# MuellerNico/DD2360-RayTracing

Hardware: AMD Instinct MI355X
Metric: Msamples/s (W*H*spp/render_time) at 1200x800, 10000 spheres (higher is better)
Workload: dtype f32

## Files before the change

dd2360-raytracing_amd/csrc/rt_kernels.hip:

```cpp
#include <hip/hip_runtime.h>
#include <float.h>
#include "rt_device.h"
#include "rt_tuning.h"
#include "rt_sampling.h"
#include "rt_sched_keep.h"

#ifdef RT_TU_CONTRACT
#pragma clang fp contract(fast)
#else
#pragma clang fp contract(off)
#endif

namespace rt {
#ifdef RT_TU_CONTRACT
namespace fmac {
#endif

#define RT_DEV static __device__ __forceinline__

#include "rt_stats.h"

struct Rng { uint32_t d, v0, v1, v2, v3, v4; };

RT_DEV float rng_uniform(Rng& s) {
// ... 185 lines not shown
                const float mn = group_min<64>(my_t);
                const int km = wave_min_int((my_t == mn && my_k != 0x7fffffff) ? my_k : 0x7fffffff);
                if (lane == L && km != 0x7fffffff && mn < closest) { closest = mn; best = T.ent_id[km]; }
            }
            return;
        }
    }
    int e_best = -1;
    int node = live ? 0 : T.n_nodes;
    const int n_nodes = T.n_nodes;
    while (true) {
        int e = 0, e_end = 0;
        while (node < n_nodes) {
            const float4 n0 = s_nodes[node * 3 + 0];
            const float4 n1 = s_nodes[node * 3 + 1];
            const float4 n2 = s_nodes[node * 3 + 2];
            const int skip = __float_as_int(n1.z);
            if (ray_box(r, n0.x, n0.y, n0.z, n0.w, n1.x, n1.y)) {
                const int cnt = __float_as_int(n2.x);
                node = node + 1;
                if (cnt > 0) { e = __float_as_int(n1.w); e_end = e + cnt; break; }
            } else {
                node = skip;
            }
        }
        if (e >= e_end) break;
        while (e < e_end) {
            const int m = e_end - e;
            const float4 s0 = T.ent_hot[e], s1 = T.ent_hot[m > 1 ? e + 1 : e], s2 = T.ent_hot[m > 2 ? e + 2 : e], s3 = T.ent_hot[m > 3 ? e + 3 : e];
            sphere_test(r, a, s0.x, s0.y, s0.z, s0.w, e, closest, e_best);
            if (m > 1) sphere_test(r, a, s1.x, s1.y, s1.z, s1.w, e + 1, closest, e_best);
            if (m > 2) sphere_test(r, a, s2.x, s2.y, s2.z, s2.w, e + 2, closest, e_best);
            if (m > 3) sphere_test(r, a, s3.x, s3.y, s3.z, s3.w, e + 3, closest, e_best);
            e += m > 4 ? 4 : m;
        }
    }
    if (e_best >= 0) best = T.ent_id[e_best];
}

RT_DEV bool eligible(const float4* s_nodes, const RayF& r, float cand, int sphere STAT_ARG) {
    const DevTree& T = cold_args()->tree;
    STAT(st, ST_ELIG, 1); WPASS(WP_ELIG_FN);
    {
        const int row = T.acc.bits_index[sphere];
        const float px = r.o.x + cand * r.d.x, py = r.o.y + cand * r.d.y, pz = r.o.z + cand * r.d.z;
        const int ix = (int)floorf((px + kRootHalfXZf) * kInvCellXZf), iy = (int)floorf(py * kInvCellYf), iz = (int)floorf((pz + kRootHalfXZf) * kInvCellXZf);
        if (row >= 0 && ix >= 0 && ix < 8 && iy >= 0 && iy < 8 && iz >= 0 && iz < 8) {
            const int cell = ix * 64 + iy * 8 + iz;
            const int node = T.acc.cellnode[cell];
            const uint32_t word = T.acc.cellbits[row * 16 + (cell >> 5)];
            if (node >= 0 && ((word >> (cell & 31)) & 1u)) {
                const float4 n0 = s_nodes[node * 3 + 0];
                const float4 n1 = s_nodes[node * 3 + 1];
                const float m = 0.012f;
                if (px > n0.x + m && px < n0.w - m && py > n0.y + m && py < n1.x - m && pz > n0.z + m && pz < n1.y - m) return true;
            }
        }
    }
    const int mb = T.acc.memb_start[sphere], me = T.acc.memb_start[sphere + 1];
    for (int k = mb; k < me; ++k) {
        const int node = T.acc.memb_cell[k];
        STAT(st, ST_ELIG_NODES, 1); WPASS(WP_ELIG_LIST);
        const float4 n0 = s_nodes[node * 3 + 0];
        const float4 n1 = s_nodes[node * 3 + 1];
        if (ray_box(r, n0.x, n0.y, n0.z, n0.w, n1.x, n1.y)) return true;
    }
    return false;
}

RT_DEV bool in_brick(const RayF& r, float cand, const float4 blo, const float4 bhi) {
    const float ux = __builtin_fmaf(__builtin_fmaf(cand, r.d.x, r.o.x), kInvCellXZf, 4.0f);
    const float uy = __builtin_fmaf(cand, r.d.y, r.o.y) * kInvCellYf;
    const float uz = __builtin_fmaf(__builtin_fmaf(cand, r.d.z, r.o.z), kInvCellXZf, 4.0f);
    return ux > blo.x && ux < bhi.x && uy > blo.y && uy < bhi.y && uz > blo.z && uz < bhi.z;
}

RT_DEV void offer(const DevTree& T, const float4* s_nodes, const RayF& r, float cand, const float4 blo, const float4 bhi, float& best_t, int& best, bool& tie STAT_ARG) {
    STAT(st, ST_OFFERS, 1);
    const int id = __float_as_int(blo.w);
    if (cand < best_t) {
        bool ok = in_brick(r, cand, blo, bhi);
        if (!ok) {
            const int node1 = __float_as_int(bhi.w);
            if (node1 >= 0) {
                STAT(st, ST_ELIG, 1); STAT(st, ST_ELIG_NODES, 1); WPASS(WP_OFFER_RAYBOX);
                const float4 n0 = s_nodes[node1 * 3 + 0];
                const float4 n1 = s_nodes[node1 * 3 + 1];
                ok = ray_box(r, n0.x, n0.y, n0.z, n0.w, n1.x, n1.y);
            } else {
                ok = eligible(s_nodes, r, cand, id STAT_PASS);
            }
        }
        if (ok) { best_t = cand; best = id; }
    } else if (cand == best_t && id != best && best > 0) {
        tie = true;
    }
}

struct Walk {
    int i, iend, coff;
    float om_c, on_c, slope, dm_c;
    bool fwd, walking;
    unsigned work, cols;
};

RT_DEV void walk_clip(Walk& W, const DevAccel& A, float best_t) {
    const float fG = (float)A.G, back_c = 2e-3f * A.inv_h;
    const float pm = fminf(fmaxf(W.om_c + best_t * W.dm_c, -4.0f), fG + 4.0f);
    if (W.fwd) W.iend = min(W.iend, (int)floorf(pm + back_c) + 1);
    else W.iend = max(W.iend, (int)ceilf(pm - back_c - 1.0f) - 1);
    if (W.fwd ? (W.i >= W.iend) : (W.i <= W.iend)) W.i = W.iend;
}

RT_DEV Walk walk_setup(const DevAccel& A, const RayF& r, float best_t, int best) {
    Walk W;
    W.work = 0u; W.cols = 0u;
    const int G = A.G;
    const float fG = (float)G;
    const float slack = 2e-3f;
    const bool xmajor = fabsf(r.d.x) >= fabsf(r.d.z);
    const float om = xmajor ? r.o.x : r.o.z, on = xmajor ? r.o.z : r.o.x;
    const float dm = xmajor ? r.d.x : r.d.z, dn = xmajor ? r.d.z : r.d.x;
    W.coff = xmajor ? 0 : A.zoff;
    W.om_c = (om - A.g0) * A.inv_h; W.on_c = (on - A.g0) * A.inv_h;
    W.dm_c = dm * A.inv_h;
    const float s_c = slack * A.inv_h;
    const float rmy = W.dm_c * __builtin_amdgcn_rcpf(r.d.y);
    const float mA = W.om_c + (A.ylo - r.o.y) * rmy, mB = W.om_c + (A.yhi - r.o.y) * rmy;
    float mlo = fminf(mA, mB) - s_c, mhi = fmaxf(mA, mB) + s_c;
    W.fwd = dm > 0.0f;
    if (W.fwd) mlo = fmaxf(mlo, W.om_c - s_c); else mhi = fminf(mhi, W.om_c + s_c);
    int ilo = (int)floorf(fminf(fmaxf(mlo, -1.0f), fG)), ihi = (int)floorf(fminf(fmaxf(mhi, -1.0f), fG));
    W.walking = !(ihi < 0 || ilo > G - 1 || !(mlo <= mhi));
    ilo = max(ilo, 0); ihi = min(ihi, G - 1);
    W.i = W.fwd ? ilo : ihi;
    W.iend = (W.fwd ? ihi : ilo) + (W.fwd ? 1 : -1);
    W.slope = dn * __builtin_amdgcn_rcpf(dm);
    if (best >= 0) walk_clip(W, A, best_t);
    if (W.i == W.iend || (W.fwd ? (W.i > W.iend) : (W.i < W.iend))) W.walking = false;
    return W;
}

static_assert(RT_POOL_COLS_THIN >= RT_POOL_COLS, "a thin round takes at least as many columns as a full one");
constexpr int kWalkPool = 64 * RT_POOL_COLS;
constexpr int kWalkCand = 128;
struct WalkLds {
    uint2 seg[kWalkPool];
    unsigned pref[kWalkPool];
    float4 ray[128];
    unsigned long long key[64];
    uint4 cq[kWalkCand];
    unsigned count, tie_lo, tie_hi, pad_;
};
struct PoolSpan { unsigned cur, end, seg_end, base, sg; int owner; RayF q; float a, abt, atm; };
RT_DEV void walk_sync() { __builtin_amdgcn_fence(__ATOMIC_SEQ_CST, "wavefront"); __builtin_amdgcn_wave_barrier(); }
RT_DEV unsigned walk_excl_scan(unsigned v, unsigned& total) {
    int x = (int)v;
    x += __builtin_amdgcn_update_dpp(0, x, 0x111, 0xf, 0xf, false);
    x += __builtin_amdgcn_update_dpp(0, x, 0x112, 0xf, 0xf, false);
    x += __builtin_amdgcn_update_dpp(0, x, 0x114, 0xf, 0xf, false);
    x += __builtin_amdgcn_update_dpp(0, x, 0x118, 0xf, 0xf, false);
    x += __builtin_amdgcn_update_dpp(0, x, 0x142, 0xa, 0xf, false);
    x += __builtin_amdgcn_update_dpp(0, x, 0x143, 0xc, 0xf, false);
    total = (unsigned)__builtin_amdgcn_readlane(x, 63);
    return (unsigned)x - v;
}

RT_DEV void pool_candidate_b(const DevTree& T, const float4* s_nodes, WalkLds& L, const uint4 c, const float4 blo, const float4 bhi STAT_ARG) {
    const int owner = (int)c.w;
    const float b = __uint_as_float(c.x), disc = __uint_as_float(c.y);
    const float4 r0 = L.ray[2 * owner], r1 = L.ray[2 * owner + 1];
    RayF q; q.o = {r0.x, r0.y, r0.z}; q.d = {r0.w, r1.x, r1.y};
    const float a = r1.z;
    const unsigned long long k0 = L.key[owner];
    const float best_t = __uint_as_float((unsigned)(k0 >> 32));
    const int best = (int)(unsigned)k0;
    const float sq = sqrtf(disc);
    float cand = __builtin_inff();
    const float t1 = (-b - sq) / a;
    if (t1 > 0.001f) cand = t1;
    else { const float t2 = (-b + sq) / a; if (t2 > 0.001f) cand = t2; }
    if (!(cand <= best_t)) return;
    const int id = __float_as_int(blo.w);
    STAT(st, ST_OFFERS, 1);
    bool tie = false;
    if (cand < best_t) {
        bool ok = in_brick(q, cand, blo, bhi);
        if (!ok) {
            const int node1 = __float_as_int(bhi.w);
            if (node1 >= 0) {
                const float4 n0 = s_nodes[node1 * 3 + 0], n1 = s_nodes[node1 * 3 + 1];
                ok = ray_box(q, n0.x, n0.y, n0.z, n0.w, n1.x, n1.y);
            } else ok = eligible(s_nodes, q, cand, id STAT_PASS);
        }
        if (ok) {
            const unsigned long long old = atomicMin(&L.key[owner], ((unsigned long long)__float_as_uint(cand) << 32) | (unsigned)id);
            tie = (unsigned)(old >> 32) == __float_as_uint(cand) && (int)(unsigned)old != id && (int)(unsigned)old > 0;
        }
    } else tie = id != best && best > 0;
    if (tie) { if (owner < 32) atomicOr(&L.tie_lo, 1u << owner); else atomicOr(&L.tie_hi, 1u << (owner - 32)); }
}

RT_DEV void pool_candidate(const DevTree& T, const float4* s_nodes, WalkLds& L, const uint4 c STAT_ARG) {
    const int e = (int)c.z;
    const float4 blo = T.acc.brick[2 * e], bhi = T.acc.brick[2 * e + 1];
    pool_candidate_b(T, s_nodes, L, c, blo, bhi STAT_PASS);
}

RT_DEV void pool_drain(const DevTree& T, const float4* s_nodes, WalkLds& L, int lane, unsigned& qn STAT_ARG) {
    walk_sync();
    const unsigned cnt = min(qn, (unsigned)kWalkCand);
    for (unsigned base = 0; base < cnt; base += 64u) {
        STAT(st, ST_B_ROUNDS_WAVE, 1);
        const unsigned i = base + (unsigned)lane;
        if (i < cnt) { STAT(st, ST_B_LANES, 1); pool_candidate(T, s_nodes, L, L.cq[i] STAT_PASS); }
    }
    qn = 0u;
    walk_sync();
}

template <int RT_QUORUM_DEN>
RT_DEV void walk_pool(const DevTree& T, const float4* s_nodes, WalkLds& L, const RayF& r, float a, Walk& W, float& best_t, int& best, bool& tie STAT_ARG) {
    const DevAccel& A = T.acc;
    const int32_t* __restrict__ cs = A.cs;
    const float4* __restrict__ hot = A.hot;
    const int lane = threadIdx.x & 63;
    const int Gf = A.Gf;
    const float fF = (float)A.F, fGf = (float)Gf, fGfm = fGf - 0.5f, q_c = A.rq_c;
    const int step = W.fwd ? 1 : -1;
    const float f_atm = a * (0.001f * 0.9999f - 1e-6f);
    bool walking = W.walking && W.i != W.iend;
    const int nw0 = __popcll(__ballot(walking));
    L.ray[2 * lane] = make_float4(r.o.x, r.o.y, r.o.z, r.d.x);
    while (true) {
        L.ray[2 * lane + 1] = make_float4(r.d.y, r.d.z, a, __builtin_fmaf(a * best_t, 1.0001f, 1e-6f * a));
        L.key[lane] = ((unsigned long long)__float_as_uint(best_t) << 32) | (unsigned)best;
        if (lane == 0) { L.tie_lo = 0u; L.tie_hi = 0u; }
        walk_sync();
        const int cols_now = nw0 * RT_POOL_COLS_THIN <= kWalkPool ? RT_POOL_COLS_THIN : RT_POOL_COLS;
        int e0[RT_POOL_COLS_THIN], e1[RT_POOL_COLS_THIN];
#pragma unroll
        for (int c = 0; c < RT_POOL_COLS_THIN; ++c) {
            e0[c] = 0; e1[c] = 0;
            if (c < cols_now && walking && W.i != W.iend) {
                STAT(st, ST_COLS, 1);
                const float u0 = W.on_c + ((float)W.i - W.om_c) * W.slope, u1 = u0 + W.slope;
                const float lo = (fminf(u0, u1) - q_c) * fF, hi = (fmaxf(u0, u1) + q_c) * fF;
                if (hi >= 0.0f && lo < fGf) {
                    const int k0 = (int)fmaxf(lo, 0.0f), k1 = (int)fminf(hi, fGfm);
                    const unsigned cbase = (unsigned)(W.coff + W.i * Gf);
                    e0[c] = cs[cbase + (unsigned)k0]; e1[c] = cs[cbase + (unsigned)k1 + 1u];
                }
                W.i += step; ++W.cols;
            }
        }
        unsigned n_seg = 0u;
#pragma unroll
        for (int c = 0; c < RT_POOL_COLS_THIN; ++c) {
            if (c >= RT_POOL_COLS && c >= cols_now) break;
            const bool has = e1[c] > e0[c];
            const unsigned long long m = __ballot(has);
            if (has) {
                const unsigned slot = n_seg + __builtin_amdgcn_mbcnt_hi((unsigned)(m >> 32), __builtin_amdgcn_mbcnt_lo((unsigned)m, 0u));
                L.seg[slot] = make_uint2((unsigned)e0[c], (unsigned)(e1[c] - e0[c]) | ((unsigned)lane << 26));
                W.work += (unsigned)(e1[c] - e0[c]);
            }
            n_seg += (unsigned)__popcll(m);
        }
        walk_sync();
        if (n_seg != 0u) {
            unsigned total = 0u;
            {
                unsigned run = 0u;
#pragma unroll
                for (int k = 0; k < RT_POOL_COLS; ++k) {
                    const unsigned sidx = (unsigned)(k * 64 + lane);
                    const unsigned cnt = sidx < n_seg ? (L.seg[sidx].y & 0x3ffffffu) : 0u;
                    unsigned tot;
                    const unsigned ex = walk_excl_scan(cnt, tot);
                    if (sidx < n_seg) L.pref[sidx] = run + ex;
                    run += tot;
                }
                total = run;
            }
            walk_sync();
            const unsigned C = (total + 64u * RT_POOL_SPANS - 1u) / (64u * RT_POOL_SPANS);
            PoolSpan sp[RT_POOL_SPANS];
#pragma unroll
            for (int j = 0; j < RT_POOL_SPANS; ++j) {
                PoolSpan& S = sp[j];
                const unsigned begin = min((unsigned)(lane + 64 * j) * C, total);
                S.end = min(begin + C, total); S.cur = begin; S.seg_end = begin; S.base = 0u; S.sg = 0u; S.owner = -1;
                S.q.o = {0.f, 0.f, 0.f}; S.q.d = {0.f, 1.f, 0.f}; S.a = 1.0f; S.abt = 0.0f; S.atm = 0.0f;
                if (n_seg <= 4u) {
                    const unsigned p1 = L.pref[min(1u, n_seg - 1u)], p2 = L.pref[min(2u, n_seg - 1u)], p3 = L.pref[min(3u, n_seg - 1u)];
                    S.sg = (n_seg > 1u && p1 <= begin ? 1u : 0u) + (n_seg > 2u && p2 <= begin ? 1u : 0u) + (n_seg > 3u && p3 <= begin ? 1u : 0u);
                } else if (begin < S.end) {
                    unsigned lo = 0u, hi = n_seg;
#pragma unroll
                    for (int it = 0; it < 8; ++it) {
                        const unsigned mid = (lo + hi) >> 1;
                        if (hi - lo > 1u) { if (L.pref[mid] <= begin) lo = mid; else hi = mid; }
                    }
                    S.sg = lo;
                }
            }
            unsigned qn = 0u;
            if (RT_POOL_DIRECT && RT_POOL_SPANS == 1 && total <= 64u) {
                PoolSpan& S = sp[0];
                const bool act = S.cur < S.end;
                STAT(st, ST_A_ITERS_WAVE, 1);
                unsigned he = 0u;
                if (act) {
                    const uint2 sd = L.seg[S.sg];
                    const unsigned p0 = L.pref[S.sg];
                    he = sd.x - p0 + S.cur;
                    S.owner = (int)(sd.y >> 26);
                    const float4 r0 = L.ray[2 * S.owner], r1 = L.ray[2 * S.owner + 1];
                    S.q.o = {r0.x, r0.y, r0.z}; S.q.d = {r0.w, r1.x, r1.y}; S.a = r1.z; S.abt = r1.w;
                    S.atm = S.a * (0.001f * 0.9999f - 1e-6f);
                }
                const float4 s4 = hot[he], blo = A.brick[2 * he], bhi = A.brick[2 * he + 1];
                STAT(st, ST_TESTS, act ? 1 : 0); STAT(st, ST_A_LANE_STEPS, act ? 1 : 0);
                const float ocx = S.q.o.x - s4.x, ocy = S.q.o.y - s4.y, ocz = S.q.o.z - s4.z;
                const float b = ocx * S.q.d.x + ocy * S.q.d.y + ocz * S.q.d.z;
                const float c = (ocx * ocx + ocy * ocy + ocz * ocz) - s4.w;
                const float disc = b * b - S.a * c;
                const float ab = fabsf(b);
                const float Lm = __builtin_fmaf(ab, -1e-4f, -b) - S.abt, M = __builtin_fmaf(ab, -1e-4f, b) + S.atm;
                const float P = fmaxf(Lm, M);
                if (act && disc > 0.0f && !(P > 0.0f && P * P > disc * 1.0003f)) {
                    STAT(st, ST_DISCPOS, 1);
                    pool_candidate_b(T, s_nodes, L, make_uint4(__float_as_uint(b), __float_as_uint(disc), he, (unsigned)S.owner), blo, bhi STAT_PASS);
                }
            } else
            while (true) {
                bool any = false;
#pragma unroll
                for (int j = 0; j < RT_POOL_SPANS; ++j) any = any || sp[j].cur < sp[j].end;
                if (__ballot(any) == 0ull) break;
                STAT(st, ST_A_ITERS_WAVE, 1);
                bool act[RT_POOL_SPANS]; unsigned he[RT_POOL_SPANS]; float4 s4[RT_POOL_SPANS];
#pragma unroll
                for (int j = 0; j < RT_POOL_SPANS; ++j) {
                    PoolSpan& S = sp[j];
                    act[j] = S.cur < S.end;
                    if (act[j] && S.cur >= S.seg_end) {
                        const uint2 sd = L.seg[S.sg];
                        const unsigned p0 = L.pref[S.sg];
                        ++S.sg;
                        S.seg_end = p0 + (sd.y & 0x3ffffffu);
                        S.base = sd.x - p0;
                        const int ow = (int)(sd.y >> 26);
                        if (ow != S.owner) {
                            S.owner = ow;
                            const float4 r0 = L.ray[2 * ow], r1 = L.ray[2 * ow + 1];
                            S.q.o = {r0.x, r0.y, r0.z}; S.q.d = {r0.w, r1.x, r1.y}; S.a = r1.z; S.abt = r1.w;
                            S.atm = S.a * (0.001f * 0.9999f - 1e-6f);
                        }
                    }
                    he[j] = act[j] ? S.base + S.cur : 0u;
                    s4[j] = hot[he[j]];
                }
                bool hold[RT_POOL_SPANS]; float hb[RT_POOL_SPANS], hd[RT_POOL_SPANS];
                bool anyhold = false;
#pragma unroll
                for (int j = 0; j < RT_POOL_SPANS; ++j) {
                    const PoolSpan& S = sp[j];
                    STAT(st, ST_TESTS, act[j] ? 1 : 0); STAT(st, ST_A_LANE_STEPS, act[j] ? 1 : 0);
                    const float ocx = S.q.o.x - s4[j].x, ocy = S.q.o.y - s4[j].y, ocz = S.q.o.z - s4[j].z;
                    const float b = ocx * S.q.d.x + ocy * S.q.d.y + ocz * S.q.d.z;
                    const float c = (ocx * ocx + ocy * ocy + ocz * ocz) - s4[j].w;
                    const float disc = b * b - S.a * c;
                    const float ab = fabsf(b);
                    const float Lm = __builtin_fmaf(ab, -1e-4f, -b) - S.abt, M = __builtin_fmaf(ab, -1e-4f, b) + S.atm;
                    const float P = fmaxf(Lm, M);
                    hold[j] = act[j] && disc > 0.0f && !(P > 0.0f && P * P > disc * 1.0003f);
                    hb[j] = b; hd[j] = disc;
                    anyhold = anyhold || hold[j];
                    if (act[j]) ++sp[j].cur;
                }
                if (__ballot(anyhold) != 0ull) {
#pragma unroll
                    for (int j = 0; j < RT_POOL_SPANS; ++j) {
                        const unsigned long long hm = __ballot(hold[j]);
                        if (hm != 0ull) {
                            const unsigned slot = qn + __builtin_amdgcn_mbcnt_hi((unsigned)(hm >> 32), __builtin_amdgcn_mbcnt_lo((unsigned)hm, 0u));
                            if (hold[j]) {
                                STAT(st, ST_DISCPOS, 1);
                                const uint4 ce = make_uint4(__float_as_uint(hb[j]), __float_as_uint(hd[j]), he[j], (unsigned)sp[j].owner);
                                if (slot < (unsigned)kWalkCand) L.cq[slot] = ce;
                                else pool_candidate(T, s_nodes, L, ce STAT_PASS);
                            }
                            qn += (unsigned)__popcll(hm);
                        }
                    }
                }
                if (qn >= 64u) pool_drain(T, s_nodes, L, lane, qn STAT_PASS);
            }
            pool_drain(T, s_nodes, L, lane, qn STAT_PASS);
            (void)f_atm;
            const unsigned long long k = L.key[lane];
            best_t = __uint_as_float((unsigned)(k >> 32)); best = (int)(unsigned)k;
            const unsigned tmask = lane < 32 ? L.tie_lo : L.tie_hi;
            if ((tmask >> (lane & 31)) & 1u) tie = true;
        }
        if (walking && best >= 0) walk_clip(W, A, best_t);
        walking = walking && W.i != W.iend;
        const int left = __popcll(__ballot(walking));
        if (left == 0) break;
        if (RT_QUORUM_DEN > 0 && nw0 >= RT_QUORUM_MIN && left * RT_QUORUM_DEN <= nw0) break;
    }
    W.walking = walking;
}

template <int RT_QUORUM_DEN>
RT_DEV void walk_pool_dense(const DevTree& T, const float4* s_nodes, WalkLds& L, const RayF& r, float a, Walk& W, float& best_t, int& best, bool& tie STAT_ARG) {
    constexpr int PB = RT_DENSE_PB;
    const DevAccel& A = T.acc;
    const int32_t* __restrict__ cs = A.cs;
    const float4* __restrict__ hot = A.hot;
    const int lane = threadIdx.x & 63;
    const int Gf = A.Gf;
    const float fF = (float)A.F, fGf = (float)Gf, fGfm = fGf - 0.5f, q_c = A.rq_c;
    const int step = W.fwd ? 1 : -1;
    bool walking = W.walking && W.i != W.iend;
    const int nw0 = __popcll(__ballot(walking));
    L.ray[2 * lane] = make_float4(r.o.x, r.o.y, r.o.z, r.d.x);
    while (true) {
        L.ray[2 * lane + 1] = make_float4(r.d.y, r.d.z, a, __builtin_fmaf(a * best_t, 1.0001f, 1e-6f * a));
        L.key[lane] = ((unsigned long long)__float_as_uint(best_t) << 32) | (unsigned)best;
        if (lane == 0) { L.tie_lo = 0u; L.tie_hi = 0u; }
        walk_sync();
        int e0 = 0, e1 = 0;
        if (walking && W.i != W.iend) {
            STAT(st, ST_COLS, 1);
            const float u0 = W.on_c + ((float)W.i - W.om_c) * W.slope, u1 = u0 + W.slope;
            const float lo = (fminf(u0, u1) - q_c) * fF, hi = (fmaxf(u0, u1) + q_c) * fF;
            if (hi >= 0.0f && lo < fGf) {
                const int k0 = (int)fmaxf(lo, 0.0f), k1 = (int)fminf(hi, fGfm);
                const unsigned cbase = (unsigned)(W.coff + W.i * Gf);
                e0 = cs[cbase + (unsigned)k0]; e1 = cs[cbase + (unsigned)k1 + 1u];
            }
            W.i += step; ++W.cols;
        }
        const bool has = e1 > e0;
        const unsigned long long m = __ballot(has);
        const unsigned n_seg = (unsigned)__popcll(m);
        if (has) {
            const unsigned slot = __builtin_amdgcn_mbcnt_hi((unsigned)(m >> 32), __builtin_amdgcn_mbcnt_lo((unsigned)m, 0u));
            L.seg[slot] = make_uint2((unsigned)e0, (unsigned)(e1 - e0) | ((unsigned)lane << 26));
            W.work += (unsigned)(e1 - e0);
        }
        walk_sync();
        if (n_seg != 0u) {
            unsigned total;
            {
                const unsigned cnt = (unsigned)lane < n_seg ? (L.seg[lane].y & 0x3ffffffu) : 0u;
                const unsigned ex = walk_excl_scan(cnt, total);
                if ((unsigned)lane < n_seg) L.pref[lane] = ex;
            }
            walk_sync();
            const unsigned C = (total + 63u) / 64u;
            PoolSpan S;
            const unsigned begin = min((unsigned)lane * C, total);
            S.end = min(begin + C, total); S.cur = begin; S.seg_end = begin; S.base = 0u; S.sg = 0u; S.owner = lane;
            S.q.o = {0.f, 0.f, 0.f}; S.q.d = {0.f, 1.f, 0.f}; S.a = 1.0f; S.abt = 0.0f; S.atm = 0.0f;
            if (begin < S.end) {
                unsigned lo = 0u, hi = n_seg;
#pragma unroll
                for (int it = 0; it < 6; ++it) {
                    const unsigned mid = (lo + hi) >> 1;
                    if (hi - lo > 1u) { if (L.pref[mid] <= begin) lo = mid; else hi = mid; }
                }
                S.sg = lo;
            }
            unsigned qn = 0u;
            while (true) {
                const bool act = S.cur < S.end;
                if (__ballot(act) == 0ull) break;
                STAT(st, ST_A_ITERS_WAVE, 1);
                if (act && S.cur >= S.seg_end) {
                    const uint2 sd = L.seg[S.sg];
                    const unsigned p0 = L.pref[S.sg];
                    ++S.sg;
                    S.seg_end = p0 + (sd.y & 0x3ffffffu);
                    S.base = sd.x - p0;
                    S.owner = (int)(sd.y >> 26);
                    const float4 r0 = L.ray[2 * S.owner], r1 = L.ray[2 * S.owner + 1];
                    S.q.o = {r0.x, r0.y, r0.z}; S.q.d = {r0.w, r1.x, r1.y}; S.a = r1.z;
                    S.atm = S.a * (0.001f * 0.9999f - 1e-6f);
                }
                const unsigned nb = act ? min((unsigned)PB, min(S.seg_end, S.end) - S.cur) : 0u;
                const unsigned he0 = act ? S.base + S.cur : 0u;
                const float4* __restrict__ hp = hot + he0;
                float4 s4[PB];
#pragma unroll
                for (int k = 0; k < PB; ++k) s4[k] = hp[k];
                const float bt_now = __uint_as_float((unsigned)(L.key[S.owner] >> 32));
                S.abt = __builtin_fmaf(S.a * bt_now, 1.0001f, 1e-6f * S.a);
                if (act) { STAT(st, ST_TESTS, nb); STAT(st, ST_A_LANE_STEPS, 1); }
                bool hold[PB]; float hb[PB], hd[PB];
                bool anyhold = false;
#pragma unroll
                for (int k = 0; k < PB; ++k) {
                    const float ocx = S.q.o.x - s4[k].x, ocy = S.q.o.y - s4[k].y, ocz = S.q.o.z - s4[k].z;
                    const float b = ocx * S.q.d.x + ocy * S.q.d.y + ocz * S.q.d.z;
                    const float c = (ocx * ocx + ocy * ocy + ocz * ocz) - s4[k].w;
                    const float disc = b * b - S.a * c;
                    const float ab = fabsf(b);
                    const float Lm = __builtin_fmaf(ab, -1e-4f, -b) - S.abt, M = __builtin_fmaf(ab, -1e-4f, b) + S.atm;
                    const float P = fmaxf(Lm, M);
                    hold[k] = (unsigned)k < nb && disc > 0.0f && !(P > 0.0f && P * P > disc * 1.0003f);
                    hb[k] = b; hd[k] = disc;
                    anyhold = anyhold || hold[k];
                }
                if (__ballot(anyhold) != 0ull) {
#pragma unroll
                    for (int k = 0; k < PB; ++k) {
                        const unsigned long long hm = __ballot(hold[k]);
                        if (hm != 0ull) {
                            const unsigned slot = qn + __builtin_amdgcn_mbcnt_hi((unsigned)(hm >> 32), __builtin_amdgcn_mbcnt_lo((unsigned)hm, 0u));
                            if (hold[k]) {
                                STAT(st, ST_DISCPOS, 1);
                                const uint4 ce = make_uint4(__float_as_uint(hb[k]), __float_as_uint(hd[k]), he0 + (unsigned)k, (unsigned)S.owner);
                                if (slot < (unsigned)kWalkCand) L.cq[slot] = ce;
                                else pool_candidate(T, s_nodes, L, ce STAT_PASS);
                            }
                            qn += (unsigned)__popcll(hm);
                        }
                    }
                }
                S.cur += nb;
                if (qn >= (unsigned)RT_DENSE_DRAIN) pool_drain(T, s_nodes, L, lane, qn STAT_PASS);
            }
            pool_drain(T, s_nodes, L, lane, qn STAT_PASS);
            const unsigned long long k = L.key[lane];
            best_t = __uint_as_float((unsigned)(k >> 32)); best = (int)(unsigned)k;
            const unsigned tmask = lane < 32 ? L.tie_lo : L.tie_hi;
            if ((tmask >> (lane & 31)) & 1u) tie = true;
        }
        if (walking && best >= 0) walk_clip(W, A, best_t);
        walking = walking && W.i != W.iend;
        const int left = __popcll(__ballot(walking));
        if (left == 0) break;
        if (RT_QUORUM_DEN > 0 && nw0 >= RT_QUORUM_MIN && left * RT_QUORUM_DEN <= nw0) break;
    }
    W.walking = walking;
}

constexpr int kHotLarge = 8;
constexpr int kHotSlots = 1 + 3 * kHotLarge;
RT_DEV float4* hot_spheres(const float4* s_nodes, int n_nodes) { return (float4*)((WalkLds*)(s_nodes + n_nodes * 3) + 4); }
template <bool POOL>
// ... 1348 lines not shown
```

dd2360-raytracing_amd/csrc/rt_stats.h:

```cpp
#pragma once
#ifdef RT_STATS
enum { ST_RAYS, ST_FAST, ST_SLOW, ST_TIE, ST_COLS, ST_TESTS, ST_DISCPOS, ST_OFFERS, ST_ELIG, ST_ELIG_NODES, ST_A_ITERS_WAVE, ST_B_ROUNDS_WAVE,
       ST_LOOP_ITERS_WAVE, ST_A_LANE_STEPS, ST_B_LANES, ST_SAMPLES, ST_LIVE_GE56, ST_LIVE_32, ST_LIVE_8, ST_LIVE_LT8, ST_SWITCHES,
       ST_CYC_TOTAL, ST_CYC_CLOSEST, ST_CYC_WALK_A, ST_CYC_WALK_B, ST_CYC_SCAN, ST_CYC_SHADE, ST_REALTIME,
       ST_SPARE0, ST_SPARE1, ST_SPARE2, ST_SPARE3, ST_SPARE4, ST_SPARE5, ST_SPARE6,
       WP_GROUND, WP_LARGE_K, WP_LARGE_EXACT, WP_OFFER_NODE, WP_OFFER_RAYBOX, WP_ELIG_FN, WP_ELIG_LIST, WP_SETUP, WP_A_COL, WP_A_BATCH, WP_A_HOLD,
       WP_B_OFFER, WP_B_CLIP, WP_COOP_CHUNK, WP_SCAN, WP_SC_ANY, WP_SC_LAMB, WP_SC_METAL, WP_SC_DIEL, WP_REJ_ITER, WP_PRIMARY, WP_DISK_ITER, WP_SKY, WP_ENDPIX,
       TH_GROUND, TH_LARGE_SETUP, TH_WALK, TH_SCAN, ST_N };
#ifdef RT_STATS_LIGHT
#define TICK() 0ull
#else
#define TICK() ((unsigned long long)__builtin_amdgcn_s_memtime())
#endif
__device__ unsigned long long g_stats[ST_N];
__device__ int g_pilot_dbg[1 << 20];
__device__ unsigned long long g_wave_dbg[8192 * 4];
struct Stats { unsigned int c[ST_N]; unsigned long long cyc[8]; };
#ifdef RT_STATS_LIGHT
#define STAT(st, k, v) ((void)0)
#else
#define STAT(st, k, v) ((st).c[k] += (v))
#endif
constexpr int kWpBlocks = WP_ENDPIX - WP_GROUND + 1;
__device__ unsigned long long g_wp_cls[4 * kWpBlocks];
#ifdef RT_STATS_WPASS
__shared__ int s_wp_cls[4];
#define WPASS(k) do { const int l_ = (int)(threadIdx.x & 63); if (__builtin_amdgcn_readfirstlane(l_) == l_) { atomicAdd(&g_stats[k], 1ull); \
    atomicAdd(&g_wp_cls[(s_wp_cls[(threadIdx.x >> 6) & 3] & 3) * kWpBlocks + ((k) - WP_GROUND)], 1ull); } } while (0)
#define WPASS_CLASS(c) do { const int l_ = (int)(threadIdx.x & 63); if (__builtin_amdgcn_readfirstlane(l_) == l_) s_wp_cls[(threadIdx.x >> 6) & 3] = (c); } while (0)
#else
#define WPASS(k) ((void)0)
#define WPASS_CLASS(c) ((void)0)
#endif
#define STAT_ARG , Stats& st
#define STAT_PASS , st
#define RT_STATS_ONLY(...) __VA_ARGS__
#define RT_STATS_READERS \
hipError_t read_pilot_dbg(int* out, int n) { return hipMemcpyFromSymbol(out, HIP_SYMBOL(g_pilot_dbg), sizeof(int) * (size_t)(n < (1 << 20) ? n : (1 << 20))); } \
hipError_t read_wave_dbg(unsigned long long* out) { return hipMemcpyFromSymbol(out, HIP_SYMBOL(g_wave_dbg), sizeof(unsigned long long) * 8192 * 4); } \
hipError_t read_wp_classes(unsigned long long* out, int reset) { \
    hipError_t e = hipMemcpyFromSymbol(out, HIP_SYMBOL(g_wp_cls), sizeof(unsigned long long) * 4 * kWpBlocks); \
    if (e != hipSuccess) return e; \
    if (reset) { unsigned long long z[4 * kWpBlocks] = {0}; e = hipMemcpyToSymbol(HIP_SYMBOL(g_wp_cls), z, sizeof(z)); } \
    return e; \
} \
hipError_t read_stats(unsigned long long* out, int reset) { \
    hipError_t e = hipMemcpyFromSymbol(out, HIP_SYMBOL(g_stats), sizeof(unsigned long long) * ST_N); \
    if (e != hipSuccess) return e; \
    if (reset) { unsigned long long z[ST_N] = {0}; e = hipMemcpyToSymbol(HIP_SYMBOL(g_stats), z, sizeof(z)); } \
    return e; \
}
#else
#define STAT(st, k, v) ((void)0)
#define WPASS(k) ((void)0)
#define WPASS_CLASS(c) ((void)0)
#define STAT_ARG
#define STAT_PASS
#define RT_STATS_ONLY(...)
#define RT_STATS_READERS
#endif
```

dd2360-raytracing_amd/csrc/rt_tuning.h:

```cpp
#pragma once

#ifndef RT_RENDER_WAVES
#define RT_RENDER_WAVES 4
#endif

#ifndef RT_LONG_RATE
#define RT_LONG_RATE 14
#endif
#ifndef RT_LONG_RATE_DENSE
#define RT_LONG_RATE_DENSE 20
#endif
#ifndef RT_LONG_CHECK
#define RT_LONG_CHECK 4
#endif
#ifndef RT_F_INFLIGHT
#define RT_F_INFLIGHT 1.35f
#endif
#ifndef RT_F_INFLIGHT_DENSE
#define RT_F_INFLIGHT_DENSE 1.1f
#endif

#ifndef RT_F_STATIC
#define RT_F_STATIC 1.07f
#endif
#ifndef RT_HEAD_SUM_SPARSE
#define RT_HEAD_SUM_SPARSE 1
#endif
#ifndef RT_HEAD_SUM_DENSE
#define RT_HEAD_SUM_DENSE -21
#endif
#ifndef RT_HEAD_LOAD_DENSE
#define RT_HEAD_LOAD_DENSE 3500
#endif
#ifndef RT_F_TAIL
#define RT_F_TAIL 0.15f
#endif
#ifndef RT_INTERLEAVE
#define RT_INTERLEAVE 64
#endif
#ifndef RT_INTERLEAVE_DENSE
#define RT_INTERLEAVE_DENSE 16
#endif
#ifndef RT_INTERLEAVE_SOLO
#define RT_INTERLEAVE_SOLO 1
#endif
#ifndef RT_LONG_RATE_MIN
#define RT_LONG_RATE_MIN 8
#endif
#ifndef RT_PILOT_LONG_SUM_MIN
#define RT_PILOT_LONG_SUM_MIN 120
#endif
#ifndef RT_MED_RATE
#define RT_MED_RATE 12
#endif
#ifndef RT_THIN_CAP_DEN
#define RT_THIN_CAP_DEN 4
#endif
#ifndef RT_LONG_PER_WAVE
#define RT_LONG_PER_WAVE 16
#endif
#ifndef RT_PILOT_SAMPLES
#define RT_PILOT_SAMPLES 2
#endif
#ifndef RT_PILOT_LONG_SUM
#define RT_PILOT_LONG_SUM 200
#endif
#ifndef RT_SOLO_DENSITY
#define RT_SOLO_DENSITY 1.0
#endif
#ifndef RT_PILOT_SOLO_SUM
#define RT_PILOT_SOLO_SUM 200
#endif
#ifndef RT_PILOT_CAP
#define RT_PILOT_CAP 35
#endif
#ifndef RT_SCHED_CACHE
#define RT_SCHED_CACHE 1
#endif
#ifndef RT_PROG_OWN
#define RT_PROG_OWN 64
#endif

#ifndef RT_SPLIT_WB
#define RT_SPLIT_WB 1000
#endif
#ifndef RT_SPLIT_WT
#define RT_SPLIT_WT 17
#endif
#ifndef RT_SPLIT_WC
#define RT_SPLIT_WC 0
#endif

#ifndef RT_ACCEL_FINE
#define RT_ACCEL_FINE 8
#endif
#ifndef RT_DENSE_CELL
#define RT_DENSE_CELL 0.7
#endif
#ifndef RT_SPARSE_CELL
#define RT_SPARSE_CELL 1.0
#endif

#ifndef RT_QUORUM_SPARSE
#define RT_QUORUM_SPARSE 4
#endif
#ifndef RT_QUORUM_DENSE
#define RT_QUORUM_DENSE 2
#endif
#ifndef RT_QUORUM_MIN
#define RT_QUORUM_MIN 16
#endif
#ifndef RT_POOL_COLS
#define RT_POOL_COLS 2
#endif
#ifndef RT_POOL_COLS_THIN
#define RT_POOL_COLS_THIN 4
#endif
#ifndef RT_POOL_SPANS
#define RT_POOL_SPANS 1
#endif
#ifndef RT_POOL_DIRECT
#define RT_POOL_DIRECT 1
#endif
#ifndef RT_DENSE_PB
#define RT_DENSE_PB 4
#endif
#ifndef RT_DENSE_DRAIN
#define RT_DENSE_DRAIN 32
#endif

#ifndef RT_LIST_BATCH
#define RT_LIST_BATCH 8
#endif
#ifndef RT_LIST_COOP_COST
#define RT_LIST_COOP_COST 16
#endif

#ifndef RT_H16_MINWAVES
#define RT_H16_MINWAVES 4
#endif
#ifndef RT_H16_BIG
#define RT_H16_BIG 128
#endif
#ifndef RT_H16_SMALL
#define RT_H16_SMALL 256
#endif
#ifndef RT_H16_INTERLEAVE
#define RT_H16_INTERLEAVE 64
#endif
#ifndef RT_H16_TASKS
#define RT_H16_TASKS 384
#endif
#ifndef RT_H16_PP
#define RT_H16_PP 10
#endif
#ifndef RT_H16_LONG_PER_WAVE
#define RT_H16_LONG_PER_WAVE 16
#endif
#ifndef RT_H16_LONG_RATE
#define RT_H16_LONG_RATE 14
#endif
#ifndef RT_H16_LONG_CHECK
#define RT_H16_LONG_CHECK 4
#endif
#ifndef RT_H16_THIN_CAP_DEN
#define RT_H16_THIN_CAP_DEN 4
#endif
#ifndef RT_H16_PILOT_LONG_SUM
#define RT_H16_PILOT_LONG_SUM 150
#endif
#ifndef RT_H16_PILOT_CAP
#define RT_H16_PILOT_CAP 35
#endif
```

Before: 4746.

## Add thin-round walk path spreading few walkers' columns across all lanes

When a wave has at most 16 active walkers, each walker's four grid columns are now given to separate lanes (16 walkers x 4 columns), so the cell-start lookups happen in parallel instead of each walker looping over its own columns. If the combined candidate count fits in 64, candidates are handed out one per lane and tested right away, skipping the segment/span pooling machinery. Otherwise it falls back to building segments. It also stops scanning empty second segment pages and passes ray data directly to the candidate routine. This adds LDS record traffic and extra branches, and carries a risk around correctness of the iteration bookkeeping.

```diff
diff --git a/dd2360-raytracing_amd/csrc/rt_kernels.hip b/dd2360-raytracing_amd/csrc/rt_kernels.hip
--- a/dd2360-raytracing_amd/csrc/rt_kernels.hip
+++ b/dd2360-raytracing_amd/csrc/rt_kernels.hip
@@ -361,6 +361,10 @@
     uint4 cq[kWalkCand];
     unsigned count, tie_lo, tie_hi, pad_;
 };
+constexpr int kThinWalkers = 16, kThinCols = 4;
+static_assert(kThinWalkers * kThinCols == 64, "a thin round: one lane per (walker, column)");
+static_assert(kThinCols == RT_POOL_COLS_THIN, "a thin round takes the columns a round of few walkers took before it");
+static_assert(sizeof(unsigned) * kWalkPool >= sizeof(uint4) * 2 * kThinWalkers && sizeof(uint2) * kWalkPool >= sizeof(uint2) * 64, "the thin round's records and slots live in pref and seg");
 struct PoolSpan { unsigned cur, end, seg_end, base, sg; int owner; RayF q; float a, abt, atm; };
 RT_DEV void walk_sync() { __builtin_amdgcn_fence(__ATOMIC_SEQ_CST, "wavefront"); __builtin_amdgcn_wave_barrier(); }
 RT_DEV unsigned walk_excl_scan(unsigned v, unsigned& total) {
@@ -375,12 +379,9 @@
     return (unsigned)x - v;
 }
 
-RT_DEV void pool_candidate_b(const DevTree& T, const float4* s_nodes, WalkLds& L, const uint4 c, const float4 blo, const float4 bhi STAT_ARG) {
+RT_DEV void pool_candidate_b(const DevTree& T, const float4* s_nodes, WalkLds& L, const uint4 c, const RayF& q, const float a, const float4 blo, const float4 bhi STAT_ARG) {
     const int owner = (int)c.w;
     const float b = __uint_as_float(c.x), disc = __uint_as_float(c.y);
-    const float4 r0 = L.ray[2 * owner], r1 = L.ray[2 * owner + 1];
-    RayF q; q.o = {r0.x, r0.y, r0.z}; q.d = {r0.w, r1.x, r1.y};
-    const float a = r1.z;
     const unsigned long long k0 = L.key[owner];
     const float best_t = __uint_as_float((unsigned)(k0 >> 32));
     const int best = (int)(unsigned)k0;
@@ -413,7 +414,9 @@
 RT_DEV void pool_candidate(const DevTree& T, const float4* s_nodes, WalkLds& L, const uint4 c STAT_ARG) {
     const int e = (int)c.z;
     const float4 blo = T.acc.brick[2 * e], bhi = T.acc.brick[2 * e + 1];
-    pool_candidate_b(T, s_nodes, L, c, blo, bhi STAT_PASS);
+    const float4 r0 = L.ray[2 * c.w], r1 = L.ray[2 * c.w + 1];
+    RayF q; q.o = {r0.x, r0.y, r0.z}; q.d = {r0.w, r1.x, r1.y};
+    pool_candidate_b(T, s_nodes, L, c, q, r1.z, blo, bhi STAT_PASS);
 }
 
 RT_DEV void pool_drain(const DevTree& T, const float4* s_nodes, WalkLds& L, int lane, unsigned& qn STAT_ARG) {
@@ -440,12 +443,95 @@
     const float f_atm = a * (0.001f * 0.9999f - 1e-6f);
     bool walking = W.walking && W.i != W.iend;
     const int nw0 = __popcll(__ballot(walking));
+    const bool thin_round = RT_POOL_THIN_ROUND && nw0 <= kThinWalkers;
     L.ray[2 * lane] = make_float4(r.o.x, r.o.y, r.o.z, r.d.x);
     while (true) {
         L.ray[2 * lane + 1] = make_float4(r.d.y, r.d.z, a, __builtin_fmaf(a * best_t, 1.0001f, 1e-6f * a));
         L.key[lane] = ((unsigned long long)__float_as_uint(best_t) << 32) | (unsigned)best;
         if (lane == 0) { L.tie_lo = 0u; L.tie_hi = 0u; }
+        const unsigned long long wmask = __ballot(walking);
+        if (thin_round && walking) {
+            const unsigned rank = __builtin_amdgcn_mbcnt_hi((unsigned)(wmask >> 32), __builtin_amdgcn_mbcnt_lo((unsigned)wmask, 0u));
+            uint4* rec = (uint4*)L.pref;
+            rec[2 * rank] = make_uint4((unsigned)lane, (unsigned)W.i, (unsigned)step, (unsigned)W.iend);
+            rec[2 * rank + 1] = make_uint4(__float_as_uint(W.om_c), __float_as_uint(W.on_c), __float_as_uint(W.slope), (unsigned)W.coff);
+        }
         walk_sync();
+        unsigned n_seg = 0u;
+        bool picked = false;
+        bool dealt = false;
+        if (thin_round) {
+            const int nwr = __popcll(wmask);
+            const int wk = lane >> 2, c = lane & 3;
+            int f0 = 0; unsigned cnt = 0u;
+            if (wk < nwr) {
+                const uint4* rec = (const uint4*)L.pref;
+                const uint4 ra = rec[2 * wk], rb = rec[2 * wk + 1];
+                const int wstep = (int)ra.z;
+                if (c < ((int)ra.w - (int)ra.y) * wstep) {
+                    const int wi = (int)ra.y + c * wstep;
+                    const float w_om = __uint_as_float(rb.x), w_on = __uint_as_float(rb.y), w_slope = __uint_as_float(rb.z);
+                    const float u0 = w_on + ((float)wi - w_om) * w_slope, u1 = u0 + w_slope;
+                    const float lo = (fminf(u0, u1) - q_c) * fF, hi = (fmaxf(u0, u1) + q_c) * fF;
+                    if (hi >= 0.0f && lo < fGf) {
+                        const int k0 = (int)fmaxf(lo, 0.0f), k1 = (int)fminf(hi, fGfm);
+                        const unsigned cbase = (unsigned)((int)rb.w + wi * Gf);
+                        const int a0 = cs[cbase + (unsigned)k0], a1 = cs[cbase + (unsigned)k1 + 1u];
+                        if (a1 > a0) { f0 = a0; cnt = (unsigned)(a1 - a0); }
+                    }
+                }
+            }
+            int qs = (int)cnt;
+            qs += __builtin_amdgcn_update_dpp(0, qs, 0xB1, 0xf, 0xf, false);
+            qs += __builtin_amdgcn_update_dpp(0, qs, 0x4E, 0xf, 0xf, false);
+            const unsigned rank = __builtin_amdgcn_mbcnt_hi((unsigned)(wmask >> 32), __builtin_amdgcn_mbcnt_lo((unsigned)wmask, 0u));
+            const int mywork = __builtin_amdgcn_ds_bpermute((int)((rank & 15u) << 4), qs);
+            if (walking) {
+                const int taken = min(kThinCols, (W.iend - W.i) * step);
+                STAT(st, ST_COLS, taken);
+                W.i += taken * step; W.cols += (unsigned)taken; W.work += (unsigned)mywork;
+            }
+            unsigned total;
+            const unsigned ex = walk_excl_scan(cnt, total);
+            RT_STATS_ONLY(n_seg = (unsigned)__popcll(__ballot(cnt != 0u)); TRSTAT_ROUND(lane, n_seg, total); n_seg = 0u;)
+            if (total <= 64u) {
+                dealt = true;
+                if (total != 0u) {
+                    picked = true;
+                    uint2* slot = (uint2*)L.seg;
+#pragma nounroll
+                    for (unsigned t = 0u; t < cnt; ++t) slot[ex + t] = make_uint2((unsigned)f0 + t, L.pref[8 * wk]);
+                    walk_sync();
+                    const bool act = (unsigned)lane < total;
+                    STAT(st, ST_A_ITERS_WAVE, 1);
+                    unsigned he = 0u; int owner = 0;
+                    if (act) { const uint2 sl = slot[lane]; he = sl.x; owner = (int)sl.y; }
+                    const float4 r0 = L.ray[2 * owner], r1 = L.ray[2 * owner + 1];
+                    const float4 s4 = hot[he], blo = A.brick[2 * he], bhi = A.brick[2 * he + 1];
+                    RayF q; q.o = {r0.x, r0.y, r0.z}; q.d = {r0.w, r1.x, r1.y};
+                    const float qa = r1.z, abt = r1.w, atm = qa * (0.001f * 0.9999f - 1e-6f);
+                    STAT(st, ST_TESTS, act ? 1 : 0); STAT(st, ST_A_LANE_STEPS, act ? 1 : 0);
+                    const float ocx = q.o.x - s4.x, ocy = q.o.y - s4.y, ocz = q.o.z - s4.z;
+                    const float b = ocx * q.d.x + ocy * q.d.y + ocz * q.d.z;
+                    const float cc = (ocx * ocx + ocy * ocy + ocz * ocz) - s4.w;
+                    const float disc = b * b - qa * cc;
+                    const float ab = fabsf(b);
+                    const float Lm = __builtin_fmaf(ab, -1e-4f, -b) - abt, M = __builtin_fmaf(ab, -1e-4f, b) + atm;
+                    const float P = fmaxf(Lm, M);
+                    if (act && disc > 0.0f && !(P > 0.0f && P * P > disc * 1.0003f)) {
+                        STAT(st, ST_DISCPOS, 1);
+                        pool_candidate_b(T, s_nodes, L, make_uint4(__float_as_uint(b), __float_as_uint(disc), he, (unsigned)owner), q, qa, blo, bhi STAT_PASS);
+                    }
+                    walk_sync();
+                }
+            } else {
+                const bool has = cnt != 0u;
+                const unsigned long long m = __ballot(has);
+                if (has) L.seg[__builtin_amdgcn_mbcnt_hi((unsigned)(m >> 32), __builtin_amdgcn_mbcnt_lo((unsigned)m, 0u))] = make_uint2((unsigned)f0, cnt | (L.pref[8 * wk] << 26));
+                n_seg = (unsigned)__popcll(m);
+                walk_sync();
+            }
+        } else {
         const int cols_now = nw0 * RT_POOL_COLS_THIN <= kWalkPool ? RT_POOL_COLS_THIN : RT_POOL_COLS;
         int e0[RT_POOL_COLS_THIN], e1[RT_POOL_COLS_THIN];
 #pragma unroll
@@ -463,7 +549,6 @@
                 W.i += step; ++W.cols;
             }
         }
-        unsigned n_seg = 0u;
 #pragma unroll
         for (int c = 0; c < RT_POOL_COLS_THIN; ++c) {
             if (c >= RT_POOL_COLS && c >= cols_now) break;
@@ -477,12 +562,16 @@
             n_seg += (unsigned)__popcll(m);
         }
         walk_sync();
-        if (n_seg != 0u) {
+        RT_STATS_ONLY(if (nw0 <= kThinWalkers && n_seg == 0u) TRSTAT_ROUND(lane, 0u, 0u);)
+        }
+        if (!dealt && n_seg != 0u) {
+            picked = true;
             unsigned total = 0u;
             {
                 unsigned run = 0u;
 #pragma unroll
                 for (int k = 0; k < RT_POOL_COLS; ++k) {
+                    if (k > 0 && n_seg <= 64u * (unsigned)k) break;
                     const unsigned sidx = (unsigned)(k * 64 + lane);
                     const unsigned cnt = sidx < n_seg ? (L.seg[sidx].y & 0x3ffffffu) : 0u;
                     unsigned tot;
@@ -492,6 +581,7 @@
                 }
                 total = run;
             }
+            RT_STATS_ONLY(if (nw0 <= kThinWalkers && !thin_round) TRSTAT_ROUND(lane, n_seg, total);)
             walk_sync();
             const unsigned C = (total + 64u * RT_POOL_SPANS - 1u) / (64u * RT_POOL_SPANS);
             PoolSpan sp[RT_POOL_SPANS];
@@ -540,7 +630,7 @@
                 const float P = fmaxf(Lm, M);
                 if (act && disc > 0.0f && !(P > 0.0f && P * P > disc * 1.0003f)) {
                     STAT(st, ST_DISCPOS, 1);
-                    pool_candidate_b(T, s_nodes, L, make_uint4(__float_as_uint(b), __float_as_uint(disc), he, (unsigned)S.owner), blo, bhi STAT_PASS);
+                    pool_candidate_b(T, s_nodes, L, make_uint4(__float_as_uint(b), __float_as_uint(disc), he, (unsigned)S.owner), S.q, S.a, blo, bhi STAT_PASS);
                 }
             } else
             while (true) {
@@ -609,6 +699,8 @@
             }
             pool_drain(T, s_nodes, L, lane, qn STAT_PASS);
             (void)f_atm;
+        }
+        if (picked) {
             const unsigned long long k = L.key[lane];
             best_t = __uint_as_float((unsigned)(k >> 32)); best = (int)(unsigned)k;
             const unsigned tmask = lane < 32 ? L.tie_lo : L.tie_hi;
diff --git a/dd2360-raytracing_amd/csrc/rt_stats.h b/dd2360-raytracing_amd/csrc/rt_stats.h
--- a/dd2360-raytracing_amd/csrc/rt_stats.h
+++ b/dd2360-raytracing_amd/csrc/rt_stats.h
@@ -6,7 +6,8 @@
        ST_SPARE0, ST_SPARE1, ST_SPARE2, ST_SPARE3, ST_SPARE4, ST_SPARE5, ST_SPARE6,
        WP_GROUND, WP_LARGE_K, WP_LARGE_EXACT, WP_OFFER_NODE, WP_OFFER_RAYBOX, WP_ELIG_FN, WP_ELIG_LIST, WP_SETUP, WP_A_COL, WP_A_BATCH, WP_A_HOLD,
        WP_B_OFFER, WP_B_CLIP, WP_COOP_CHUNK, WP_SCAN, WP_SC_ANY, WP_SC_LAMB, WP_SC_METAL, WP_SC_DIEL, WP_REJ_ITER, WP_PRIMARY, WP_DISK_ITER, WP_SKY, WP_ENDPIX,
-       TH_GROUND, TH_LARGE_SETUP, TH_WALK, TH_SCAN, ST_N };
+       TH_GROUND, TH_LARGE_SETUP, TH_WALK, TH_SCAN,
+       TR_ROUNDS, TR_SEG0, TR_SEG1, TR_SEG4, TR_SEG16, TR_SEGMORE, TR_LE64, ST_N };
 #ifdef RT_STATS_LIGHT
 #define TICK() 0ull
 #else
@@ -18,8 +19,12 @@
 struct Stats { unsigned int c[ST_N]; unsigned long long cyc[8]; };
 #ifdef RT_STATS_LIGHT
 #define STAT(st, k, v) ((void)0)
+#define TRSTAT_ROUND(lane, n_seg, total) ((void)0)
 #else
 #define STAT(st, k, v) ((st).c[k] += (v))
+#define TRSTAT_ROUND(lane, n_seg, total) do { if ((lane) == 0) { atomicAdd(&g_stats[TR_ROUNDS], 1ull); \
+    atomicAdd(&g_stats[(n_seg) == 0u ? TR_SEG0 : (n_seg) == 1u ? TR_SEG1 : (n_seg) <= 4u ? TR_SEG4 : (n_seg) <= 16u ? TR_SEG16 : TR_SEGMORE], 1ull); \
+    if ((total) <= 64u) atomicAdd(&g_stats[TR_LE64], 1ull); } } while (0)
 #endif
 constexpr int kWpBlocks = WP_ENDPIX - WP_GROUND + 1;
 __device__ unsigned long long g_wp_cls[4 * kWpBlocks];
diff --git a/dd2360-raytracing_amd/csrc/rt_tuning.h b/dd2360-raytracing_amd/csrc/rt_tuning.h
--- a/dd2360-raytracing_amd/csrc/rt_tuning.h
+++ b/dd2360-raytracing_amd/csrc/rt_tuning.h
@@ -116,6 +116,9 @@
 #ifndef RT_POOL_COLS_THIN
 #define RT_POOL_COLS_THIN 4
 #endif
+#ifndef RT_POOL_THIN_ROUND
+#define RT_POOL_THIN_ROUND 1
+#endif
 #ifndef RT_POOL_SPANS
 #define RT_POOL_SPANS 1
 #endif
```

After: 4830, median of 6. 1.8% higher.
